# roryhighnam/iib_project_ldpc_codes

Hardware: AMD Instinct MI355X
Metric: decoded codewords/sec + info-bit Gb/s, (3,6) n=10k 50-iter BP, 1/2/4/8 MI355X (higher is better)
Workload: dtype f32

## Files before the change

iib_project_ldpc_codes_amd/_native.py:

```python
import ctypes as ct
import os

HERE = os.path.dirname(os.path.abspath(__file__))
LIB_PATH = os.environ.get("LDPC_LIB_PATH") or os.path.join(HERE, "libldpc_mi355x.so")

LDPC_OK = 0
LDPC_EINVAL, LDPC_ENODEV, LDPC_EHIP, LDPC_ENOMEM, LDPC_EUNSUP = -1, -2, -3, -4, -5
CH_BEC, CH_BSC, CH_AWGN = 0, 1, 2
ALGO_SPA, ALGO_MINSUM = 0, 1
MC_NCOUNT = 4
RM_TX, RM_PUNCT, RM_KNOWN = 0, 1, 2

_lib = None


class Quant(ct.Structure):
    _fields_ = [("scale", ct.c_float), ("msg_bits", ct.c_int32), ("post_bits", ct.c_int32),
                ("norm8", ct.c_int32), ("offset", ct.c_int32)]


class LdpcError(RuntimeError):
    def __init__(self, func, rc, msg):
        super().__init__(f"{func} failed ({rc}): {msg}")
        self.rc = rc
# ... 24 lines not shown
    "ldpc_bp_decode_batch_dev": ([P, P, i, i, i, f, i, P, P, P, P], i),
    "ldpc_channel_dev": ([i, f, u64, u64, i, i, P, P], i),
    "ldpc_mc_batch_dev": ([P, i, f, u64, u64, i, i, i, f, i, i, i64, P, P], i),
    "ldpc_last_error": ([], ct.c_char_p),
    "ldpc_device_count": ([], i),
    "ldpc_set_device": ([i], i),
    "ldpc_sync": ([P], i),
    "ldpc_bp_kernel_name": ([P, i], ct.c_char_p),
    "ldpc_debug_lane_layout": ([P, P, i, i, i, i, P, P, P, P], i),
    "ldpc_debug_irr_layout": ([P, P, P, P, i, i, P, P, P], i),
    "ldpc_debug_loc_layout": ([P, P, P, P, i, i, i, P, P, P, P], i),
    "ldpc_debug_loc_chain_layout": ([P, P, P, P, i, i, P, P, P, P, P], i),
    "ldpc_debug_loc_variant": ([P, P, P, P, i, i, i, P], i),
    "ldpc_debug_mc_plan": ([P, i64, i64, i64, i, i, P], i),
    "ldpc_debug_bp_plan": ([P, P, P, P, i, i, i, P, i, P, P], i),
    "ldpc_bp_layered_decode_batch_dev": ([P, P, i, i, i, f, i, P, P, P, P], i),
    "ldpc_mc_layered_batch_dev": ([P, i, f, u64, u64, i, i, i, f, i, i, i64, P, P], i),
    "ldpc_debug_layer_schedule": ([P, P, P, P, i, i, P, P], i),
    "ldpc_layer_rule": ([], ct.c_char_p),
    "ldpc_debug_layer_plan": ([P, P, P, P, i, i, i, P, i, P, P], i),
    "ldpc_bp_layered_q_decode_batch_dev": ([P, P, i, i, P, i, P, P, P, P], i),
    "ldpc_mc_layered_q_batch_dev": ([P, i, f, u64, u64, i, i, P, i, i, i64, P, P], i),
    "ldpc_debug_layer_q_plan": ([P, P, P, P, i, i, i, P, i, P, P], i),
    "ldpc_mc_layered_q_cw_batch_dev": ([P, P, P, i, f, f, u64, u64, i, i, P, i, i, i64, P, P], i),
    "ldpc_debug_layer_q_cw_plan": ([P, P, P, P, i, i, i, P, i, i, P, P], i),
    "ldpc_debug_qc_cw_plan": ([i, i, i, P, i, P, i, i, P, P], i),
    "ldpc_quant_check": ([P], i),
    "ldpc_graph_create_qc": ([i, i, i, P, ct.POINTER(P)], i),
    "ldpc_graph_layer_rule": ([P], ct.c_char_p),
    "ldpc_debug_qc_expand": ([i, i, i, P, P, P, P, P, P], i),
# ... 70 lines not shown
```

iib_project_ldpc_codes_amd/csrc/bp_dispatch.hip:

```cpp
#include "kernel_args.hpp"
#include "ldpc_mi355x.h"

namespace ldpc {

int device_cus() {
    int dev = 0, cus = 0;
    if (hipGetDevice(&dev) != hipSuccess ||
        hipDeviceGetAttribute(&cus, hipDeviceAttributeMultiprocessorCount, dev) != hipSuccess || cus <= 0)
        cus = 256;
    return cus;
}

const char *bp_kernel_name(const ldpc_graph &g, int early_stop) {
    return bp_plan(g, 1, 50, 0, early_stop != 0, false, early_stop != 2, device_cus()).name;
}

hipError_t FloodFamily::launch(const BpPlan &p, const SoftCall &c, float *scratch, hipStream_t s) const {
    BpArgs a = call_args<BpArgs>(c);
    a.cptr = g.cptr;
    a.cvar = g.cvar;
    a.vptr = g.vptr;
    a.vslot = g.vslot;
    a.n = g.n;
    a.m = g.m;
    a.E = g.E;
    a.scratch = scratch;
    a.scratch_bytes = p.scratch;
    const bool et = c.early_stop, mc = c.mc;
    switch (p.path) {
        case BpPath::Loc: return c.algo == 0 ? launch_loc_spa(p, g, a, et, mc, s) : launch_loc_ms(p, g, a, et, mc, s);
        case BpPath::Lds36: return launch_lds36(p, g, a, c.algo, et, mc, s);
        case BpPath::Irr: return launch_irr(p, g, a, c.algo, et, mc, s);
        case BpPath::None: return hipErrorInvalidValue;
        default: return launch_generic(p, g, a, c.algo, et, mc, s);
    }
}

hipError_t LayerFamily::launch(const BpPlan &p, const SoftCall &c, float *scratch, hipStream_t s) const {
    if (p.path == BpPath::None || !g.lay_tab || !g.lay_var) return hipErrorNotSupported;
    LayerArgs a = call_args<LayerArgs>(c);
    a.tab = g.lay_tab;
    a.var = g.lay_var;
// ... 40 lines not shown
```

iib_project_ldpc_codes_amd/csrc/bp_loc.hpp:

```cpp
#pragma once
#include "bp_device.hpp"

namespace ldpc {
namespace {

#ifndef LDPC_LOC_VGROUP
#define LDPC_LOC_VGROUP 1
#endif
#ifndef LDPC_LOC_CGROUP
#define LDPC_LOC_CGROUP 1
#endif
template <int N, int D>
__device__ __forceinline__ uint32_t bits_parity(const float2 (&x)[D], bool hi, uint32_t seed) {
    auto w = [&](int j) { return __float_as_uint(hi ? x[j].y : x[j].x); };
    uint32_t p = seed;
    int j = 2;
#pragma unroll
    for (; j + 1 < N; j += 2) p = xor3u(p, w(j), w(j + 1));
    if (j < N) p ^= w(j);
    return p;
}
template <int D, int ALGO, bool MIXED = false, bool SGN = false, int CL = 0>
__device__ __forceinline__ int loc_check_pair(float *msg, int W, int Nc, int i, float2 &l0, float2 &l1, float alpha,
                                              uint32_t lpar = 0u, float2 *chain = nullptr) {
// ... 53 lines not shown
__device__ __forceinline__ int loc_check_dispatch(int code, float *msg, int W, int Nc, int i, float2 &l0, float2 &l1,
                                                  float alpha, uint32_t lpar) {
    if constexpr (D == DHI) {
        if (code >> 8) return loc_check_pair<D, ALGO, true, SGN>(msg, W, Nc, i, l0, l1, alpha, lpar);
        return loc_check_pair<D, ALGO, false, SGN>(msg, W, Nc, i, l0, l1, alpha, lpar);
    } else {
        if (code == D) return loc_check_pair<D, ALGO, false, SGN>(msg, W, Nc, i, l0, l1, alpha, lpar);
        return loc_check_dispatch<D + 1, DHI, ALGO, SGN>(code, msg, W, Nc, i, l0, l1, alpha, lpar);
    }
}

template <typename V>
__device__ __forceinline__ V ld_fresh(const V *p, int idx) {
    asm volatile("" : "+v"(idx));
    return p[idx];
}

__device__ __forceinline__ bool block_any(int pred, uint32_t *flag, int par) {
    if (__builtin_amdgcn_ballot_w64(pred != 0) != 0 && (threadIdx.x & (kWave - 1)) == 0) flag[par] = 1u;
    __syncthreads();
    const bool any = flag[par] != 0u;
    if (threadIdx.x == 0) flag[par ^ 1] = 0u;
    return any;
}
__device__ __forceinline__ uint32_t block_count(int pred, uint32_t *flag, int par) {
    const uint64_t bal = __builtin_amdgcn_ballot_w64(pred != 0);
    if (bal != 0 && (threadIdx.x & (kWave - 1)) == 0) atomicAdd(&flag[par], (uint32_t)__popcll(bal));
    __syncthreads();
    const uint32_t c = flag[par];
    if (threadIdx.x == 0) flag[par ^ 1] = 0u;
// ... 23 lines not shown
    constexpr int VP = 2 * KP;
    constexpr int DVM = DVN0 > DVN1 ? DVN0 : DVN1;
    constexpr int DVA = DVM > 0 ? DVM : 1;
    constexpr int DVP = DVA;
    extern __shared__ __align__(16) unsigned char smem[];
    __shared__ uint32_t stop_flag[2];
    float *msg = reinterpret_cast<float *>(smem);
    const int tid = threadIdx.x;
    const int n = a.n, iters = a.max_iters;
    const int lpos0 = (int)((uint32_t)(size_t)(lds_u8 *)smem >> 2);
    const uint32_t base2 = (uint32_t)lpos0 | ((uint32_t)lpos0 << 16);
    constexpr bool SPA = ALGO == 0;
    constexpr bool INF0 = ABS0 || ALGO == 1, INF1 = ABS1 || ALGO == 1;
    uint32_t sp[VP][DVA];
    uint32_t inf[VP];
    auto load_sp = [&](int v, int u) {
        return (uint32_t)ld_fresh(a.loc_pos, (v * DVP + u) * T + tid) + base2;
    };
    auto load_vars = [&](int (&vv)[2 * VP]) {
#pragma unroll
        for (int i = 0; i < 2 * VP; ++i) vv[i] = ld_fresh(a.loc_var, i * T + tid);
    };
#pragma unroll
    for (int k = 0; k < KP; ++k) {
        if constexpr (INF0) inf[2 * k] = (uint32_t)a.loc_info[(2 * k) * T + tid];
        if constexpr (INF1) inf[2 * k + 1] = (uint32_t)a.loc_info[(2 * k + 1) * T + tid];
    }
    auto at = [](uint32_t ba) -> lds_f32 & { return *(lds_f32 *)(size_t)ba; };
    const float neutral = SPA ? 1.0f : 0.0f;

    auto gather = [&](auto dn_tag, auto abs_tag, int v, const uint32_t (&spv)[DVA], float2 (&cv)[DVA],
                      uint32_t (&a0)[DVA], uint32_t (&a1)[DVA]) {
        constexpr int DN = decltype(dn_tag)::value;
        constexpr bool AB = decltype(abs_tag)::value;
        const int nl = chained(v) ? DN - 1 : DN;
#pragma unroll
// ... 109 lines not shown
        if (per && tid == 0) next_b = round == 0 ? (int)atomicAdd(a.work, 1u) : (int)claim;
        __syncthreads();
        const int b = per ? __builtin_amdgcn_readfirstlane(next_b) : (int)blockIdx.x + round * (int)gridDim.x;
        if (b >= a.B) break;
        if (per && tid == 0) claim = atomicAdd(a.work, 1u);
        const uint64_t cw = a.first_cw + (uint64_t)b;
        int redo_it = -1;
    restart:
        int slab_it = -2;
        bool slab_now = false;
        if constexpr (ET) {
            if (tid == 0) stop_flag[0] = stop_flag[1] = 0u;
        }
        constexpr bool STG = CL > 0;
        auto load_tabs = [&]() {
#pragma unroll
            for (int k = 0; k < KP; ++k) {
#pragma unroll
                for (int u = 0; u < DVN0; ++u) sp[2 * k][u] = load_sp(2 * k, u);
#pragma unroll
                for (int u = 0; u < DVN1; ++u)
                    if (!(chained(2 * k + 1) && u == DVN1 - 1)) sp[2 * k + 1][u] = load_sp(2 * k + 1, u);
            }
        };
        int vv[2 * VP];
        if constexpr (STG) {
            load_tabs();
            load_vars(vv);
        }
        int err0 = 0;
        if constexpr (MC) {
            for (int i = tid; i <= iters; i += T) curve[i] = 0;
            if constexpr (MSET)
                for (int i = tid; i < nsw; i += T) syn[i] = 0u;
            for (int g4 = tid; g4 < (n + 3) >> 2; g4 += T) {
                const uint4 r = chan_block(a.ch, cw, g4);
#pragma unroll
                for (int q = 0; q < 4; ++q) {
                    if (4 * g4 + q >= n) break;
                    const float l = chan_soft_word(a.ch, r, q);
                    msg[4 * g4 + q] = to_msg<ALGO>(l);
                    err0 += (l < 0.0f);
                }
            }
        } else {
            if constexpr (MSET)
                for (int i = tid; i < nsw; i += T) syn[i] = 0u;
            if constexpr (STG) {
                float r[2 * VP];
                const float *lb = a.llr + (size_t)b * n;
                int t = tid;
                asm volatile("" : "+v"(t));
#pragma unroll
                for (int i = 0; i < 2 * VP; ++i) r[i] = lb[min(t + i * T, n - 1)];
#pragma unroll
                for (int i = 0; i < 2 * VP; ++i)
                    if (t + i * T < n) msg[t + i * T] = to_msg<ALGO>(r[i]);
            } else {
                for (int v = tid; v < n; v += T) msg[v] = to_msg<ALGO>(a.llr[(size_t)b * n + v]);
            }
        }
        __syncthreads();
        if constexpr (MC) {
            const int w = wave_sum(err0);
            if ((tid & (kWave - 1)) == 0) atomicAdd(&curve[0], w);
        }
        if constexpr (!STG) load_tabs();
        float2 L[VP];
        if constexpr (MC || STG) {
            if constexpr (!STG) load_vars(vv);
#pragma unroll
            for (int v = 0; v < VP; ++v)
                L[v] = make_float2(vv[2 * v] >= 0 ? msg[vv[2 * v]] : 0.0f, vv[2 * v + 1] >= 0 ? msg[vv[2 * v + 1]] : 0.0f);
        } else {
#pragma unroll
            for (int v = 0; v < VP; ++v) {
                const int v0 = ld_fresh(a.loc_var, (v * 2 + 0) * T + tid), v1 = ld_fresh(a.loc_var, (v * 2 + 1) * T + tid);
                L[v] = make_float2(v0 >= 0 ? msg[v0] : 0.0f, v1 >= 0 ? msg[v1] : 0.0f);
            }
        }
        __syncthreads();
        float2 loc[VP];
        auto init = [&](auto dn_tag, int v) {
            constexpr int DN = decltype(dn_tag)::value;
            float2 w;
// ... 264 lines not shown
                    if (v0 >= 0) msg[v0] = (hbits >> (2 * v)) & 1 ? -1.0f : 1.0f;
                    if (v1 >= 0) msg[v1] = (hbits >> (2 * v + 1)) & 1 ? -1.0f : 1.0f;
                }
                __syncthreads();
                if (a.hard)
                    for (int v = tid; v < n; v += T) a.hard[(size_t)b * n + v] = (uint8_t)(msg[v] < 0.0f);
                if (a.its && tid == 0) a.its[b] = it;
                continue;
            }
        }
        constexpr bool FIX = !ET && !MC;
        float2 pr[VP];
        int pid[2 * VP];
        bool clamped = false;
        if constexpr (FIX) {
            load_vars(pid);
            if constexpr (SPA) {
#pragma unroll
                for (int v = 0; v < VP; ++v)
                    clamped |= fabsf(__builtin_amdgcn_logf(L[v].x)) >= 125.5f || fabsf(__builtin_amdgcn_logf(L[v].y)) >= 125.5f;
            }
        }
        auto post = [&](auto dn_tag, auto abs_tag, auto subst_tag, int v) {
            constexpr int DN = decltype(dn_tag)::value;
            constexpr bool SUBST = decltype(subst_tag)::value;
            uint32_t a0[DVA], a1[DVA], spv[DVA];
            float2 cv[DVA];
            if constexpr (FIX) {
                gather(dn_tag, abs_tag, v, sp[v], cv, a0, a1);
            } else {
#pragma unroll
// ... 29 lines not shown
        };
        if (FIX && SPA && __builtin_expect(__builtin_amdgcn_ballot_w64(clamped) != 0, 0)) {
#pragma unroll
            for (int k = 0; k < KP; ++k) {
                post(int_c<DVN0>{}, bool_c<ABS0>{}, bool_c<true>{}, 2 * k);
                post(int_c<DVN1>{}, bool_c<ABS1>{}, bool_c<true>{}, 2 * k + 1);
            }
        } else {
#pragma unroll
            for (int k = 0; k < KP; ++k) {
                post(int_c<DVN0>{}, bool_c<ABS0>{}, bool_c<false>{}, 2 * k);
                post(int_c<DVN1>{}, bool_c<ABS1>{}, bool_c<false>{}, 2 * k + 1);
            }
        }
        __syncthreads();
#pragma unroll
        for (int v = 0; v < VP; ++v) {
            int v0, v1;
            if constexpr (FIX) {
                v0 = pid[2 * v];
                v1 = pid[2 * v + 1];
            } else {
                v0 = ld_fresh(a.loc_var, (v * 2 + 0) * T + tid);
                v1 = ld_fresh(a.loc_var, (v * 2 + 1) * T + tid);
            }
            if (v0 >= 0) msg[v0] = pr[v].x;
            if (v1 >= 0) msg[v1] = pr[v].y;
        }
        __syncthreads();
        if constexpr (FIX) {
            float o[2 * VP];
            int t = tid;
            asm volatile("" : "+v"(t));
#pragma unroll
            for (int i = 0; i < 2 * VP; ++i) o[i] = msg[min(t + i * T, n - 1)];
#pragma unroll
            for (int i = 0; i < 2 * VP; ++i) {
                const int v = t + i * T;
                if (v < n) {
                    if (a.post) a.post[(size_t)b * n + v] = o[i] * Domain<ALGO>::out;
                    if (a.hard) a.hard[(size_t)b * n + v] = (uint8_t)(o[i] < 0.0f);
                }
            }
        } else {
            for (int v = tid; v < n; v += T) {
                const float s = msg[v];
                if (a.post) a.post[(size_t)b * n + v] = s * Domain<ALGO>::out;
                if (a.hard) a.hard[(size_t)b * n + v] = (uint8_t)(s < 0.0f);
            }
        }
        if (a.its && tid == 0) a.its[b] = iters;
    }
}

template <int DLO, int DHI, int D0, int D1, bool A0, bool A1, int T, int KP, int ALGO, bool ET, bool MC>
hipError_t launch_loc_shape(const BpPlan &p, BpArgs a, hipStream_t s) {
// ... 78 lines not shown
```

iib_project_ldpc_codes_amd/csrc/bp_plan.cpp:

```cpp
#include "ldpc_internal.hpp"

#ifndef LDPC_LDS36_MINSUM
#define LDPC_LDS36_MINSUM 1
#endif
#ifndef LDPC_LOC
#define LDPC_LOC 1
#endif
#ifndef LDPC_LOC_CHAIN
#define LDPC_LOC_CHAIN 1
#endif
#ifndef LDPC_LOC_MSMC
#define LDPC_LOC_MSMC 1
#endif
#ifndef LDPC_LOC_HARD_ET
#define LDPC_LOC_HARD_ET 1
#endif
#ifndef LDPC_LOC_ET_POST
#define LDPC_LOC_ET_POST 1
#endif
#ifndef LDPC_LOC_PERSIST
#define LDPC_LOC_PERSIST 1
#endif
#ifndef LDPC_LDS36_GRID
#define LDPC_LDS36_GRID 256
#endif
#ifndef LDPC_GMEM_GRID
#define LDPC_GMEM_GRID 256
#endif
#ifndef LDPC_GMEM_HYB
#define LDPC_GMEM_HYB 1
#endif

namespace ldpc {
namespace {

size_t loc_lds_bytes(const GraphShape &g, int iters, bool mc, bool syn) {
    return pad16((size_t)std::max(g.loc_words + 64, g.n) * 4) + (mc ? curve_bytes(iters) : 0) +
           (syn ? (size_t)((g.m + 31) / 32) * 4 : 0);
}
size_t loc_ep_slab_bytes(const GraphShape &g) { return (size_t)(2 * g.loc_KP) * (size_t)g.loc_T * 2 * 4; }

size_t irr_lds_bytes(const GraphShape &g, int iters) {
    const int nsyn = (g.m + 31) >> 5;
    return pad16((size_t)g.irr_S * 4) + (size_t)((nsyn + 3) & ~3) * 4 + (size_t)(iters + 1) * 4;
}
bool irr_slab(const GraphShape &g) { return g.irr_S < g.irr_P; }

size_t lds36_bytes(const GraphShape &g, int iters, bool et, bool mc) {
    const size_t Ep = (size_t)lds_pair_span(g.m, 6) + kLdsDummy;
    size_t s = Ep * 4;
    if (et || mc) s = pad16(Ep * 5);
    if (mc) s += (size_t)(iters + 1) * 4;
// ... 4 lines not shown
size_t generic_lds_bytes(const GraphShape &g, int iters, bool mc) {
    return generic_msg_bytes(g) + (mc ? (size_t)(iters + 1) * 4 : 0);
}

void gmem_plan(BpPlan &p, size_t fixed, size_t E) {
    p.threads = LDPC_GMEM_T;
    const size_t room = fixed < kLdsMax - 4096 ? kLdsMax - 4096 - fixed : 0;
    p.lds_slots = LDPC_GMEM_HYB ? (int)std::min(E, room / 4) : 0;
    p.lds = fixed + (size_t)p.lds_slots * 4;
}

BpPath choose_path(const GraphShape &g, int iters, bool et, bool mc, int algo, bool hard_only) {
    if (!g.consistent) return BpPath::None;
    const bool lds36_ms = LDPC_LDS36_MINSUM && algo == 1 && g.lane_T && g.dv == 3 && g.dc == 6 && g.loc_T != 512;
    const bool one_cls = loc_variant(g) == kLocReg36;
    const bool ep_ok = LDPC_LOC_ET_POST && (size_t)std::max(g.loc_words + 64, g.n) * 4 >= (size_t)g.n * 5;
    const bool mode_ok = mc ? (algo == 0 || (LDPC_LOC_MSMC && one_cls))
                            : (!et || (LDPC_LOC_HARD_ET && (hard_only || ep_ok) && (algo == 0 || one_cls)));
    const bool mset = et && algo == 1;
    if (LDPC_LOC && mode_ok && iters > 0 && !lds36_ms && loc_variant(g) != kLocNone &&
        loc_lds_bytes(g, iters, mc || mset, mset) <= kLdsMax - 2048)
        return BpPath::Loc;
    if (g.lane_T && g.dv == 3 && g.dc == 6 && lds36_bytes(g, iters, et, mc) <= kLdsMax - 2048)
        return BpPath::Lds36;
    if (g.irr_VPT && irr_lds_bytes(g, iters) <= kLdsMax - 1024) return BpPath::Irr;
    const int d = g.max_cdeg;
    if (d > 32) return BpPath::None;
    const bool lds = generic_lds_bytes(g, iters, mc) <= kLdsMax - 2048;
    if (d <= 8) return lds ? BpPath::Generic8 : BpPath::GenericG8;
    if (d <= 16) return lds ? BpPath::Generic16 : BpPath::GenericG16;
    return lds ? BpPath::Generic32 : BpPath::GenericG32;
}

}

BpPlan bp_plan(const GraphShape &g, int B, int iters, int algo, bool et, bool mc, bool want_post, int cus) {
    algo = algo ? 1 : 0;
    BpPlan p;
    p.path = choose_path(g, iters, et, mc, algo, !want_post);
    p.grid = B;
    size_t slab_per_wg = 0;
    switch (p.path) {
        case BpPath::Loc: {
            p.name = "bp_loc_kernel";
            p.threads = g.loc_T;
            const bool mset = et && algo == 1;
            p.lds = loc_lds_bytes(g, iters, mc || mset, mset);
            p.chain = LDPC_LOC_CHAIN && g.chn_Tq > 0 && algo == 0 && !et && !mc;
            if (p.chain) p.lds = pad16((size_t)std::max(g.chn_words + 64, g.n) * 4);
            const bool ep = et && !mc && want_post;
            p.persistent = ep || ((et || LDPC_LOC_PERSIST > 1) && LDPC_LOC_PERSIST);
            if (p.persistent) p.grid = std::min(B, 2 * cus);
            if (ep) slab_per_wg = loc_ep_slab_bytes(g);
            break;
        }
        case BpPath::Lds36:
            p.name = "bp_lds_kernel<3,6>";
            p.threads = g.lane_T;
            p.lds = lds36_bytes(g, iters, et, mc);
            if (et || (LDPC_LDS36_PREFETCH && !mc)) p.grid = std::min(B, LDPC_LDS36_GRID);
            break;
        case BpPath::Irr:
            p.name = irr_slab(g) ? "bp_irr_kernel<lds+slab>" : "bp_irr_kernel<lds>";
            p.threads = kIrrT;
// ... 20 lines not shown
                                                    : "bp_generic_kernel<32,gmem>";
            p.grid = std::min(B, LDPC_GMEM_GRID);
            gmem_plan(p, mc ? curve_bytes(iters) : 0, (size_t)g.E);
            slab_per_wg = generic_msg_bytes(g);
            break;
        }
        default: return p;
    }
    p.slab = slab_per_wg * (size_t)p.grid;
    p.scratch = p.slab;
    if (p.persistent) {
        p.counter = (long)p.slab;
        p.scratch += sizeof(uint32_t);
    }
    return p;
}

BpPlan bp_ens_plan(int n, int dv, int dc, int B, int iters, int , bool , bool mc,
                   bool , int cus) {
    BpPlan p;
    if (n <= 0 || dv <= 0 || dc <= 1 || dc > 32) return p;
    const size_t E = (size_t)n * (size_t)dv;
    const size_t block = ens_block_bytes((size_t)n, E), syn = ens_syn_bytes(E / (size_t)dc);
    const bool lds = block + syn + (mc ? (size_t)(iters + 1) * 4 : 0) <= kLdsMax - 2048;
    const int w = dc <= 8 ? 0 : (dc <= 16 ? 1 : 2);
    static const BpPath paths[2][3] = {{BpPath::EnsG8, BpPath::EnsG16, BpPath::EnsG32},
                                       {BpPath::Ens8, BpPath::Ens16, BpPath::Ens32}};
    static const char *const names[2][3] = {{"bp_ens_kernel<8,gmem>", "bp_ens_kernel<16,gmem>", "bp_ens_kernel<32,gmem>"},
                                            {"bp_ens_kernel<8,lds>", "bp_ens_kernel<16,lds>", "bp_ens_kernel<32,lds>"}};
    p.grid = std::min(B, std::min(cus, LDPC_GMEM_GRID));
// ... 87 lines not shown
```

iib_project_ldpc_codes_amd/csrc/capi.cpp:

```cpp
#include <cmath>
#include <cstdio>
#include <cstdlib>
#include <algorithm>
#include <cstring>
#include <memory>
#include <mutex>
#include <string>
#include <vector>

#include "encode_host.hpp"
#include "graph_device.hpp"
#include "rate_match_host.hpp"
#include "workspace.hpp"

namespace ldpc {
namespace {
thread_local std::string g_err;
std::mutex g_mu;
DropInCache g_dropin;

LayoutOptions layout_options(int loc_T = 0) {
    LayoutOptions opt;
    const char *noloc = getenv("LDPC_NO_LOC_LAYOUT");
    opt.loc_layout = !(noloc && noloc[0] == '1');
// ... 55 lines not shown
    host_layouts(h, g, L, true, layout_options());
    if (need_schedule && g.lay_L <= 0) {
        set_error(kNoSchedule);
        return LDPC_EUNSUP;
    }
    return write_plans(count, calls, out, names, col4, no_plan,
                       [&](int B, int iters, int algo, bool et, bool mc, bool want_post) {
                           return plan(g, B, iters, algo, et, mc, want_post, cus);
                       });
}

static SoftCall decode_call(int B, int max_iters, int algo, float alpha, int early_stop, const float *llr, void *post,
                            uint8_t *hard, int32_t *its) {
    SoftCall c{B, max_iters, algo, alpha, early_stop != 0, false};
    c.llr = llr, c.post = post, c.hard = hard, c.its = its;
    return c;
}
static SoftCall mc_call(int B, int max_iters, int algo, float alpha, int early_stop, const ChanArgs &ch,
                        uint64_t first_cw) {
    SoftCall c{B, max_iters, algo, alpha, early_stop != 0, true};
    c.ch = ch, c.first_cw = first_cw;
    return c;
}

template <typename Family>
static int soft_launch(Workspace &ws, const Family &f, const SoftCall &c, hipStream_t s) {
    const BpPlan p = f.plan(c, device_cus());
    float *scratch = p.scratch ? ws.scratch.get<float>((p.scratch + 3) / 4) : nullptr;
    LDPC_ALLOCATED(scratch || !p.scratch);
    if (p.scratch > (scratch ? ws.scratch.cap : 0)) LDPC_HIP(hipErrorInvalidValue);
// ... 184 lines not shown
    LDPC_TRY(host_graph_from_csr(check_ptr, check_var, var_ptr, var_slot, n, m, h));
    *variant = kLocNone;
    if (!h.consistent) return LDPC_OK;
    GraphShape g;
    HostLayouts L;
    host_layouts(h, g, L, true, layout_options(T));
    *variant = loc_variant(g);
    return LDPC_OK;
}

int ldpc_debug_bp_plan(const int32_t *check_ptr, const int32_t *check_var, const int32_t *var_ptr,
                       const int32_t *var_slot, int n, int m, int count, const int32_t *calls, int cus, int64_t *out,
                       char *names) {
    return graph_plans(check_ptr, check_var, var_ptr, var_slot, n, m, count, calls, cus, out, names, bp_plan, false,
                       &BpPlan::lds_slots);
}

int ldpc_debug_bec_plan(int n, int m, int dc, int count, const int32_t *calls, int64_t *out, char *names) {
    LDPC_REQUIRE(n > 0 && m > 0 && dc >= 0 && count >= 0 && (count == 0 || (calls && out && names)),
                 "bad plan arguments");
    for (int i = 0; i < count; ++i) {
        const int32_t *c = calls + 4 * (size_t)i;
        LDPC_REQUIRE(c[0] >= 0 && c[0] <= 2 && c[1] >= 0 && c[2] >= 0, "bad plan arguments");
        const BecPlan p = bec_plan(n, m, dc, c[1], c[2], static_cast<BecMode>(c[0]), c[3]);
        int64_t *o = out + 9 * (size_t)i;
        o[0] = (int64_t)p.kernel; o[1] = p.threads; o[2] = p.W; o[3] = p.plane; o[4] = p.cw_per_wg;
        o[5] = p.grid; o[6] = (int64_t)p.lds; o[7] = p.F; o[8] = (int64_t)p.cap;
        snprintf(names + 64 * (size_t)i, 64, "%s", p.name);
    }
    return LDPC_OK;
// ... 977 lines not shown
```

iib_project_ldpc_codes_amd/csrc/kernel_args.hpp:

```cpp
#pragma once
#include "device_common.hpp"
#include "ldpc_internal.hpp"

namespace ldpc {

struct BecArgs {
    const int32_t *cvar, *cptr, *vptr, *vchk;
    int n, m, dv, dc;
    uint8_t *words;
    int32_t *errors, *its;
    int max_iters;
    ChanArgs ch;
    uint64_t first_cw;
    int32_t *trial;
    int64_t graph_stride;
};

struct BpArgs {
    const int32_t *cptr, *cvar, *vptr, *vslot;
    int n, m, E, B;
    const float *llr;
    float *post;
    uint8_t *hard;
    int32_t *its;
    int max_iters;
    float alpha;
    ChanArgs ch;
    uint64_t first_cw;
    int32_t *trial;
    float *scratch;
    size_t scratch_bytes;
    const int32_t *lane_var, *lane_slot;
    int lds_slots;
    const int32_t *irr_lane, *irr_cdeg;
    int irr_KC, irr_S, irr_P;
    const int32_t *loc_var, *loc_pos, *loc_info;
    int loc_P, loc_ncls, loc_words;
    int loc_cls_q[5], loc_cls_d[4], loc_cls_w[5];
    uint32_t *work;
};

struct EnsArgs {
    const int32_t *chk, *var;
    int n, m, dv, dc, E, B;
    const float *llr;
    float *post;
    uint8_t *hard;
    int32_t *its;
// ... 104 lines not shown
```

iib_project_ldpc_codes_amd/csrc/ldpc_internal.hpp:

```cpp
#pragma once
#include <hip/hip_runtime.h>
#include <stdint.h>

#include <algorithm>
#include <string>
#include <vector>

#include "kernel_shapes.hpp"

struct ldpc_quant;

struct GraphShape {
    int n = 0, m = 0, k = 0, E = 0;
    int dv = 0, dc = 0;
    int max_vdeg = 0, max_cdeg = 0;
    bool consistent = false;
    int vchk_len = 0;
    int lane_T = 0, lane_VPT = 0;
    int irr_VPT = 0, irr_KC = 0, irr_DC = 0, irr_S = 0, irr_P = 0;
    int loc_T = 0, loc_KP = 0, loc_DVN = 0, loc_P = 0, loc_ncls = 0, loc_words = 0, loc_dlo = 0, loc_dhi = 0;
    int loc_dvn0 = 0, loc_dvn1 = 0;
    bool loc_abs0 = false, loc_abs1 = false;
    int loc_cls_q[5] = {0}, loc_cls_d[4] = {0}, loc_cls_w[5] = {0};
    int chn_Tq = 0, chn_words = 0;
// ... 103 lines not shown
constexpr size_t kLdsMax = 160 * 1024;
constexpr size_t kBecWordLdsCap = kLdsMax - 1024, kPeelLdsCap = kLdsMax - 1024;
constexpr size_t kBecBitsLdsCap = kLdsMax - 4096, kBecBitsWideLdsCap = 72 * 1024;
constexpr int kLdsDummy = 3 * 32 + 4;

inline int lds_pair_pos(int slot, int dc) {
    const int c = slot / dc, j = slot % dc;
    return (c >> 1) * 2 * dc + 2 * j + (c & 1);
}
inline int lds_pair_span(int m, int dc) { return ((m + 1) / 2) * 2 * dc; }

namespace ldpc {

void set_error(const std::string &msg);
constexpr size_t pad16(size_t b) { return (b + 15) & ~(size_t)15; }

enum class BecMode { Decode, Mc, EnsMc };
enum class BecKernel { Word, DecBits, McBits, Peel, None };
struct BecPlan {
    BecKernel kernel = BecKernel::None;
    const char *name = "none";
    int threads = 0;
    int W = 0, plane = 0;
    int cw_per_wg = 0;
    int64_t grid = 0;
    size_t lds = 0;
    size_t cap = 0;
    int F = 0;
};
BecPlan bec_plan(int n, int m, int dc, int B, int iters, BecMode mode, int peel_cap);
// ... 24 lines not shown

enum class BpPath {
    Loc, Lds36, Irr, Generic8, Generic16, Generic32, GenericG8, GenericG16, GenericG32, None,
    Ens8, Ens16, Ens32, EnsG8, EnsG16, EnsG32,
    Layer8, Layer16, Layer32, LayerG8, LayerG16, LayerG32,
    LayerQ8, LayerQ16, LayerQ32,
    QcQ64x8, QcQ64x16, QcQ64x32, QcQ256x8, QcQ256x16, QcQ256x32
};
struct BpPlan {
    BpPath path = BpPath::None;
    const char *name = "none";
    int threads = 0, grid = 0;
    size_t lds = 0;
    int lds_slots = 0;
    bool chain = false;
    bool persistent = false;
    size_t slab = 0;
    long counter = -1;
    size_t scratch = 0;
    int wg_per_cu = 0;
};
BpPlan bp_plan(const GraphShape &g, int B, int iters, int algo, bool early_stop, bool mc, bool want_post, int cus);
BpPlan bp_ens_plan(int n, int dv, int dc, int B, int iters, int algo, bool early_stop, bool mc, bool want_post,
                   int cus);
BpPlan bp_layer_plan(const GraphShape &g, int B, int iters, int algo, bool early_stop, bool mc, bool want_post,
                     int cus);
BpPlan bp_layer_q_plan(const GraphShape &g, int B, int iters, int algo, bool early_stop, bool mc, bool want_post,
                       int cus);
BpPlan bp_layer_q_cw_plan(const GraphShape &g, int B, int iters, bool mc, bool cw);
constexpr size_t layer_q_plane_bytes(size_t n) { return 4 * ((n + 31) / 32); }
constexpr size_t layer_q_record_bytes(int max_cdeg) { return max_cdeg <= 16 ? 4 : 8; }
constexpr size_t layer_block_bytes(size_t n, size_t E) { return pad16((n + E) * 4); }
constexpr int kLayerMaxD = 32, kLayerTab = kLayerMaxD + 1;
constexpr int kQcRow = 1 + 2 * kLayerMaxD;
constexpr size_t ens_block_bytes(size_t n, size_t E) { return pad16(E * 8 + n * 4); }
constexpr size_t generic_block_bytes(size_t n, size_t E) { return pad16(E * 5 + n * 4); }
constexpr size_t curve_bytes(int iters) { return pad16((size_t)(iters + 1) * 4); }
// ... 12 lines not shown
    c.p2 = p2;
    c.k0 = (uint32_t)seed;
    c.k1 = (uint32_t)(seed >> 32);
    return c;
}

struct SoftCall {
    int B = 0, max_iters = 0, algo = 0;
    float alpha = 1.0f;
    bool early_stop = false;
    bool mc = false;
    const float *llr = nullptr;
    void *post = nullptr;
    uint8_t *hard = nullptr;
    int32_t *its = nullptr;
    ChanArgs ch{};
    uint64_t first_cw = 0;
    int32_t *trial = nullptr;
    bool cw_mode = false;
    const uint8_t *cw = nullptr;
    const uint8_t *rm = nullptr;
    float known_llr = 0.0f;
};

struct FloodFamily {
    const ldpc_graph &g;
    BpPlan plan(const SoftCall &c, int cus) const {
        return bp_plan(g, c.B, c.max_iters, c.algo, c.early_stop, c.mc, c.post != nullptr, cus);
    }
    hipError_t launch(const BpPlan &p, const SoftCall &c, float *scratch, hipStream_t s) const;
};
struct EnsFamily {
    int n, dv, dc;
    const int32_t *chk, *var;
    BpPlan plan(const SoftCall &c, int cus) const {
        return bp_ens_plan(n, dv, dc, c.B, c.max_iters, c.algo, c.early_stop, c.mc, c.post != nullptr, cus);
    }
    hipError_t launch(const BpPlan &p, const SoftCall &c, float *scratch, hipStream_t s) const;
};
struct LayerFamily {
    const ldpc_graph &g;
    BpPlan plan(const SoftCall &c, int cus) const {
        return bp_layer_plan(g, c.B, c.max_iters, c.algo, c.early_stop, c.mc, c.post != nullptr, cus);
// ... 125 lines not shown
```

iib_project_ldpc_codes_amd/csrc/loc_layout.cpp:

```cpp
#include <algorithm>
#include <cmath>
#include <cstdlib>
#include <cstdint>
#include <deque>
#include <vector>

#include "ldpc_internal.hpp"

#ifndef LDPC_LOC_SEARCH
#define LDPC_LOC_SEARCH 10
#endif
#ifndef LDPC_LOC_T0
#define LDPC_LOC_T0 0.0
#endif

namespace {
bool assign(const std::vector<std::vector<int>> &adj, std::vector<int> cap, int NR, std::vector<int> &to) {
    const int NL = (int)adj.size();
    std::vector<std::vector<int>> held(NR);
    std::vector<int> order(NL);
    to.assign(NL, -1);
    for (int v = 0; v < NL; ++v) order[v] = v;
    std::stable_sort(order.begin(), order.end(), [&](int a, int b) { return adj[a].size() < adj[b].size(); });
    for (int v : order)
// ... 596 lines not shown
        uint32_t info = 0;
        int u = 0, jl = 0;
        for (int j = 0; j < DV; ++j) {
            const int e = vslot[vptr[v] + j];
            if (slot_check[e] == c) { jl = j; continue; }
            if (urow[e] < 0) continue;
            int32_t &pk = C.pos[((size_t)vi * DVN + u) * T + t];
            pk = (int32_t)(((uint32_t)pk & ~(0xFFFFu << (16 * h))) | ((uint32_t)cw[e] << (16 * h)));
            info |= 1u << (u + 4 * h);
            ++u;
        }
        info |= (uint32_t)jl << (8 + 2 * h);
        info |= 1u << (16 + 4 * h + jl);
        C.info[(size_t)vi * T + t] |= (int32_t)info;
    }
    return true;
}
```

include/ldpc_mi355x.h:

```cpp
#ifndef LDPC_MI355X_H
#define LDPC_MI355X_H

#include <stdint.h>

#ifdef __cplusplus
extern "C" {
#endif

#define LDPC_OK 0
#define LDPC_EINVAL (-1)
#define LDPC_ENODEV (-2)
#define LDPC_EHIP (-3)
#define LDPC_ENOMEM (-4)
#define LDPC_EUNSUP (-5)

#define LDPC_CH_BEC 0
#define LDPC_CH_BSC 1
#define LDPC_CH_AWGN 2

#define LDPC_ALGO_SPA 0
#define LDPC_ALGO_MINSUM 1

int message_passing(int *Mvc, int iterations, int *variable_to_check_list,
                    int *check_to_variable_list, int *errors, int n, int k, int dv, int dc);
// ... 154 lines not shown
int ldpc_debug_irr_layout(const int32_t *check_ptr, const int32_t *check_var, const int32_t *var_ptr,
                          const int32_t *var_slot, int n, int m, int32_t *shape, int32_t *lane, int32_t *cdeg);

int ldpc_debug_loc_layout(const int32_t *check_ptr, const int32_t *check_var, const int32_t *var_ptr,
                          const int32_t *var_slot, int n, int m, int T, int32_t *shape, int32_t *var, int32_t *pos,
                          int32_t *info);

int ldpc_debug_loc_chain_layout(const int32_t *check_ptr, const int32_t *check_var, const int32_t *var_ptr,
                                const int32_t *var_slot, int n, int m, int32_t *shape, int32_t *var, int32_t *pos,
                                int32_t *info, int32_t *chk);

int ldpc_debug_bp_plan(const int32_t *check_ptr, const int32_t *check_var, const int32_t *var_ptr,
                       const int32_t *var_slot, int n, int m, int count, const int32_t *calls, int cus, int64_t *out,
                       char *names);

int ldpc_debug_ens_plan(int n, int dv, int dc, int count, const int32_t *calls, int cus, int64_t *out,
                        char *names);

int ldpc_debug_layer_schedule(const int32_t *check_ptr, const int32_t *check_var, const int32_t *var_ptr,
                              const int32_t *var_slot, int n, int m, int32_t *num_layers, int32_t *layer);
const char *ldpc_layer_rule(void);

int ldpc_debug_layer_plan(const int32_t *check_ptr, const int32_t *check_var, const int32_t *var_ptr,
                          const int32_t *var_slot, int n, int m, int count, const int32_t *calls, int cus,
                          int64_t *out, char *names);

int ldpc_debug_layer_q_plan(const int32_t *check_ptr, const int32_t *check_var, const int32_t *var_ptr,
                            const int32_t *var_slot, int n, int m, int count, const int32_t *calls, int cus,
                            int64_t *out, char *names);
int ldpc_quant_check(const ldpc_quant *q);
// ... 42 lines not shown
```

Baseline: 2.567 million.

## Use buffer loads and 128-bit vectorized LLR/posterior I/O in local BP kernel

Adds a wide_io plan flag, set when the local path runs without early stop or Monte Carlo and the pointers are aligned. With it, the kernel loads LLRs and stores posteriors and hard bits as 16-byte or packed 4-byte vectors. Table reads and the remaining I/O switch to raw buffer loads and stores, whose hardware range checks replace per-element bounds branches, and active-lane guards replace per-variable sign checks. A layout check now requires the padding lanes to be exactly those at or beyond Tq, and LDS sizing requires spare slack so that clamped out-of-range stores stay in bounds. The aim is fewer memory instructions and branches at kernel entry and exit, at the cost of stricter layout and alignment conditions.

New measurement: 2.615 million, median of 6. +1.9%, better.

```diff
diff --git a/iib_project_ldpc_codes_amd/_native.py b/iib_project_ldpc_codes_amd/_native.py
--- a/iib_project_ldpc_codes_amd/_native.py
+++ b/iib_project_ldpc_codes_amd/_native.py
@@ -62,6 +62,7 @@
     "ldpc_debug_loc_variant": ([P, P, P, P, i, i, i, P], i),
     "ldpc_debug_mc_plan": ([P, i64, i64, i64, i, i, P], i),
     "ldpc_debug_bp_plan": ([P, P, P, P, i, i, i, P, i, P, P], i),
+    "ldpc_debug_bp_plan_io": ([P, P, P, P, i, i, i, P, i, P, P], i),
     "ldpc_bp_layered_decode_batch_dev": ([P, P, i, i, i, f, i, P, P, P, P], i),
     "ldpc_mc_layered_batch_dev": ([P, i, f, u64, u64, i, i, i, f, i, i, i64, P, P], i),
     "ldpc_debug_layer_schedule": ([P, P, P, P, i, i, P, P], i),
diff --git a/iib_project_ldpc_codes_amd/csrc/bp_dispatch.hip b/iib_project_ldpc_codes_amd/csrc/bp_dispatch.hip
--- a/iib_project_ldpc_codes_amd/csrc/bp_dispatch.hip
+++ b/iib_project_ldpc_codes_amd/csrc/bp_dispatch.hip
@@ -26,6 +26,7 @@
     a.E = g.E;
     a.scratch = scratch;
     a.scratch_bytes = p.scratch;
+    a.wide_io = p.wide_io;
     const bool et = c.early_stop, mc = c.mc;
     switch (p.path) {
         case BpPath::Loc: return c.algo == 0 ? launch_loc_spa(p, g, a, et, mc, s) : launch_loc_ms(p, g, a, et, mc, s);
diff --git a/iib_project_ldpc_codes_amd/csrc/bp_loc.hpp b/iib_project_ldpc_codes_amd/csrc/bp_loc.hpp
--- a/iib_project_ldpc_codes_amd/csrc/bp_loc.hpp
+++ b/iib_project_ldpc_codes_amd/csrc/bp_loc.hpp
@@ -91,6 +91,14 @@
 __device__ __forceinline__ V ld_fresh(const V *p, int idx) {
     asm volatile("" : "+v"(idx));
     return p[idx];
+}
+typedef float f32x4 __attribute__((ext_vector_type(4)));
+typedef uint32_t u32x4 __attribute__((ext_vector_type(4)));
+__device__ __forceinline__ __amdgpu_buffer_rsrc_t row_rsrc(const void *row, int bytes) {
+    return __builtin_amdgcn_make_buffer_rsrc(const_cast<void *>(row), 0, bytes, 0x00020000);
+}
+__device__ __forceinline__ int32_t ld_row(__amdgpu_buffer_rsrc_t tab, int entry, uint32_t lane_bytes) {
+    return (int32_t)__builtin_amdgcn_raw_buffer_load_b32(tab, lane_bytes, 4 * entry, 0);
 }
 
 __device__ __forceinline__ bool block_any(int pred, uint32_t *flag, int par) {
@@ -144,12 +152,22 @@
     constexpr bool INF0 = ABS0 || ALGO == 1, INF1 = ABS1 || ALGO == 1;
     uint32_t sp[VP][DVA];
     uint32_t inf[VP];
-    auto load_sp = [&](int v, int u) {
-        return (uint32_t)ld_fresh(a.loc_pos, (v * DVP + u) * T + tid) + base2;
+    auto lane_bytes = [&]() {
+        uint32_t l = 4u * (uint32_t)tid;
+        asm volatile("" : "+v"(l));
+        return l;
+    };
+    auto load_sp = [&](int v, int u, uint32_t lane4 = 0u) {
+        if constexpr (CL > 0) return (uint32_t)ld_row(row_rsrc(a.loc_pos, VP * DVP * T * 4), (v * DVP + u) * T, lane4) + base2;
+        else return (uint32_t)ld_fresh(a.loc_pos, (v * DVP + u) * T + tid) + base2;
     };
     auto load_vars = [&](int (&vv)[2 * VP]) {
 #pragma unroll
         for (int i = 0; i < 2 * VP; ++i) vv[i] = ld_fresh(a.loc_var, i * T + tid);
+    };
+    auto load_vars_row = [&](int (&vv)[2 * VP], uint32_t lane4) {
+#pragma unroll
+        for (int i = 0; i < 2 * VP; ++i) vv[i] = ld_row(row_rsrc(a.loc_var, 2 * VP * T * 4), i * T, lane4);
     };
 #pragma unroll
     for (int k = 0; k < KP; ++k) {
@@ -289,19 +307,20 @@
         }
         constexpr bool STG = CL > 0;
         auto load_tabs = [&]() {
+            const uint32_t lane4 = CL > 0 ? lane_bytes() : 0u;
 #pragma unroll
             for (int k = 0; k < KP; ++k) {
 #pragma unroll
-                for (int u = 0; u < DVN0; ++u) sp[2 * k][u] = load_sp(2 * k, u);
+                for (int u = 0; u < DVN0; ++u) sp[2 * k][u] = load_sp(2 * k, u, lane4);
 #pragma unroll
                 for (int u = 0; u < DVN1; ++u)
-                    if (!(chained(2 * k + 1) && u == DVN1 - 1)) sp[2 * k + 1][u] = load_sp(2 * k + 1, u);
+                    if (!(chained(2 * k + 1) && u == DVN1 - 1)) sp[2 * k + 1][u] = load_sp(2 * k + 1, u, lane4);
             }
         };
         int vv[2 * VP];
         if constexpr (STG) {
             load_tabs();
-            load_vars(vv);
+            load_vars_row(vv, lane_bytes());
         }
         int err0 = 0;
         if constexpr (MC) {
@@ -322,15 +341,29 @@
             if constexpr (MSET)
                 for (int i = tid; i < nsw; i += T) syn[i] = 0u;
             if constexpr (STG) {
-                float r[2 * VP];
-                const float *lb = a.llr + (size_t)b * n;
-                int t = tid;
+                const __amdgpu_buffer_rsrc_t rl = row_rsrc(a.llr + (size_t)b * n, 4 * n);
+                uint32_t t = (uint32_t)tid;
                 asm volatile("" : "+v"(t));
-#pragma unroll
-                for (int i = 0; i < 2 * VP; ++i) r[i] = lb[min(t + i * T, n - 1)];
-#pragma unroll
-                for (int i = 0; i < 2 * VP; ++i)
-                    if (t + i * T < n) msg[t + i * T] = to_msg<ALGO>(r[i]);
+                if (a.wide_io) {
+                    f32x4 r[VP / 2];
+#pragma unroll
+                    for (int j = 0; j < VP / 2; ++j)
+                        r[j] = __builtin_bit_cast(f32x4, __builtin_amdgcn_raw_buffer_load_b128(rl, 16u * (t + j * T), 0, 0));
+#pragma unroll
+                    for (int j = 0; j < VP / 2; ++j) {
+                        f32x4 w;
+                        w.x = to_msg<ALGO>(r[j].x); w.y = to_msg<ALGO>(r[j].y);
+                        w.z = to_msg<ALGO>(r[j].z); w.w = to_msg<ALGO>(r[j].w);
+                        *reinterpret_cast<f32x4 *>(msg + min(4u * (t + j * T), (uint32_t)n)) = w;
+                    }
+                } else {
+                    float r[2 * VP];
+#pragma unroll
+                    for (int i = 0; i < 2 * VP; ++i)
+                        r[i] = __uint_as_float(__builtin_amdgcn_raw_buffer_load_b32(rl, 4u * (t + i * T), 0, 0));
+#pragma unroll
+                    for (int i = 0; i < 2 * VP; ++i) msg[min(t + i * T, (uint32_t)n)] = to_msg<ALGO>(r[i]);
+                }
             } else {
                 for (int v = tid; v < n; v += T) msg[v] = to_msg<ALGO>(a.llr[(size_t)b * n + v]);
             }
@@ -342,8 +375,15 @@
         }
         if constexpr (!STG) load_tabs();
         float2 L[VP];
-        if constexpr (MC || STG) {
-            if constexpr (!STG) load_vars(vv);
+        if constexpr (STG) {
+#pragma unroll
+            for (int v = 0; v < VP; ++v) L[v] = make_float2(0.0f, 0.0f);
+            if (tid < a.loc_cls_q[1]) {
+#pragma unroll
+                for (int v = 0; v < VP; ++v) L[v] = make_float2(msg[vv[2 * v]], msg[vv[2 * v + 1]]);
+            }
+        } else if constexpr (MC) {
+            load_vars(vv);
 #pragma unroll
             for (int v = 0; v < VP; ++v)
                 L[v] = make_float2(vv[2 * v] >= 0 ? msg[vv[2 * v]] : 0.0f, vv[2 * v + 1] >= 0 ? msg[vv[2 * v + 1]] : 0.0f);
@@ -638,7 +678,7 @@
         int pid[2 * VP];
         bool clamped = false;
         if constexpr (FIX) {
-            load_vars(pid);
+            load_vars_row(pid, lane_bytes());
             if constexpr (SPA) {
 #pragma unroll
                 for (int v = 0; v < VP; ++v)
@@ -698,32 +738,70 @@
             }
         }
         __syncthreads();
-#pragma unroll
-        for (int v = 0; v < VP; ++v) {
-            int v0, v1;
-            if constexpr (FIX) {
-                v0 = pid[2 * v];
-                v1 = pid[2 * v + 1];
-            } else {
-                v0 = ld_fresh(a.loc_var, (v * 2 + 0) * T + tid);
-                v1 = ld_fresh(a.loc_var, (v * 2 + 1) * T + tid);
-            }
-            if (v0 >= 0) msg[v0] = pr[v].x;
-            if (v1 >= 0) msg[v1] = pr[v].y;
+        if constexpr (FIX && CL > 0) {
+            if (tid < a.loc_cls_q[1]) {
+#pragma unroll
+                for (int v = 0; v < VP; ++v) {
+                    msg[pid[2 * v]] = pr[v].x;
+                    msg[pid[2 * v + 1]] = pr[v].y;
+                }
+            }
+        } else if constexpr (FIX) {
+#pragma unroll
+            for (int v = 0; v < VP; ++v) {
+                msg[min((uint32_t)pid[2 * v], (uint32_t)n)] = pr[v].x;
+                msg[min((uint32_t)pid[2 * v + 1], (uint32_t)n)] = pr[v].y;
+            }
+        } else {
+#pragma unroll
+            for (int v = 0; v < VP; ++v) {
+                const int v0 = ld_fresh(a.loc_var, (v * 2 + 0) * T + tid);
+                const int v1 = ld_fresh(a.loc_var, (v * 2 + 1) * T + tid);
+                if (v0 >= 0) msg[v0] = pr[v].x;
+                if (v1 >= 0) msg[v1] = pr[v].y;
+            }
         }
         __syncthreads();
         if constexpr (FIX) {
-            float o[2 * VP];
-            int t = tid;
+            uint32_t t = (uint32_t)tid;
             asm volatile("" : "+v"(t));
-#pragma unroll
-            for (int i = 0; i < 2 * VP; ++i) o[i] = msg[min(t + i * T, n - 1)];
-#pragma unroll
-            for (int i = 0; i < 2 * VP; ++i) {
-                const int v = t + i * T;
-                if (v < n) {
-                    if (a.post) a.post[(size_t)b * n + v] = o[i] * Domain<ALGO>::out;
-                    if (a.hard) a.hard[(size_t)b * n + v] = (uint8_t)(o[i] < 0.0f);
+            if (a.wide_io) {
+                f32x4 o[VP / 2];
+#pragma unroll
+                for (int j = 0; j < VP / 2; ++j)
+                    o[j] = *reinterpret_cast<const f32x4 *>(msg + min(4u * (t + j * T), (uint32_t)n));
+                if (a.post) {
+                    const __amdgpu_buffer_rsrc_t rp = row_rsrc(a.post + (size_t)b * n, 4 * n);
+#pragma unroll
+                    for (int j = 0; j < VP / 2; ++j)
+                        __builtin_amdgcn_raw_buffer_store_b128(__builtin_bit_cast(u32x4, o[j] * Domain<ALGO>::out), rp,
+                                                               16u * (t + j * T), 0, 0);
+                }
+                if (a.hard) {
+                    const __amdgpu_buffer_rsrc_t rh = row_rsrc(a.hard + (size_t)b * n, n);
+#pragma unroll
+                    for (int j = 0; j < VP / 2; ++j) {
+                        const uint32_t h = (uint32_t)(o[j].x < 0.0f) | (uint32_t)(o[j].y < 0.0f) << 8 |
+                                           (uint32_t)(o[j].z < 0.0f) << 16 | (uint32_t)(o[j].w < 0.0f) << 24;
+                        __builtin_amdgcn_raw_buffer_store_b32(h, rh, 4u * (t + j * T), 0, 0);
+                    }
+                }
+            } else {
+                float o[2 * VP];
+#pragma unroll
+                for (int i = 0; i < 2 * VP; ++i) o[i] = msg[min(t + i * T, (uint32_t)n)];
+                if (a.post) {
+                    const __amdgpu_buffer_rsrc_t rp = row_rsrc(a.post + (size_t)b * n, 4 * n);
+#pragma unroll
+                    for (int i = 0; i < 2 * VP; ++i)
+                        __builtin_amdgcn_raw_buffer_store_b32(__float_as_uint(o[i] * Domain<ALGO>::out), rp,
+                                                              4u * (t + i * T), 0, 0);
+                }
+                if (a.hard) {
+                    const __amdgpu_buffer_rsrc_t rh = row_rsrc(a.hard + (size_t)b * n, n);
+#pragma unroll
+                    for (int i = 0; i < 2 * VP; ++i)
+                        __builtin_amdgcn_raw_buffer_store_b8((uint8_t)(o[i] < 0.0f), rh, t + i * T, 0, 0);
                 }
             }
         } else {
diff --git a/iib_project_ldpc_codes_amd/csrc/bp_plan.cpp b/iib_project_ldpc_codes_amd/csrc/bp_plan.cpp
--- a/iib_project_ldpc_codes_amd/csrc/bp_plan.cpp
+++ b/iib_project_ldpc_codes_amd/csrc/bp_plan.cpp
@@ -35,7 +35,7 @@
 namespace {
 
 size_t loc_lds_bytes(const GraphShape &g, int iters, bool mc, bool syn) {
-    return pad16((size_t)std::max(g.loc_words + 64, g.n) * 4) + (mc ? curve_bytes(iters) : 0) +
+    return pad16(loc_msg_words(g.loc_words, g.n) * 4) + (mc ? curve_bytes(iters) : 0) +
            (syn ? (size_t)((g.m + 31) / 32) * 4 : 0);
 }
 size_t loc_ep_slab_bytes(const GraphShape &g) { return (size_t)(2 * g.loc_KP) * (size_t)g.loc_T * 2 * 4; }
@@ -70,11 +70,11 @@
     if (!g.consistent) return BpPath::None;
     const bool lds36_ms = LDPC_LDS36_MINSUM && algo == 1 && g.lane_T && g.dv == 3 && g.dc == 6 && g.loc_T != 512;
     const bool one_cls = loc_variant(g) == kLocReg36;
-    const bool ep_ok = LDPC_LOC_ET_POST && (size_t)std::max(g.loc_words + 64, g.n) * 4 >= (size_t)g.n * 5;
+    const bool ep_ok = LDPC_LOC_ET_POST && loc_msg_words(g.loc_words, g.n) * 4 >= (size_t)g.n * 5;
     const bool mode_ok = mc ? (algo == 0 || (LDPC_LOC_MSMC && one_cls))
                             : (!et || (LDPC_LOC_HARD_ET && (hard_only || ep_ok) && (algo == 0 || one_cls)));
     const bool mset = et && algo == 1;
-    if (LDPC_LOC && mode_ok && iters > 0 && !lds36_ms && loc_variant(g) != kLocNone &&
+    if (LDPC_LOC && mode_ok && iters > 0 && !lds36_ms && loc_variant(g) != kLocNone && loc_spare_ok(g.loc_words, g.n) &&
         loc_lds_bytes(g, iters, mc || mset, mset) <= kLdsMax - 2048)
         return BpPath::Loc;
     if (g.lane_T && g.dv == 3 && g.dc == 6 && lds36_bytes(g, iters, et, mc) <= kLdsMax - 2048)
@@ -102,8 +102,8 @@
             p.threads = g.loc_T;
             const bool mset = et && algo == 1;
             p.lds = loc_lds_bytes(g, iters, mc || mset, mset);
-            p.chain = LDPC_LOC_CHAIN && g.chn_Tq > 0 && algo == 0 && !et && !mc;
-            if (p.chain) p.lds = pad16((size_t)std::max(g.chn_words + 64, g.n) * 4);
+            p.chain = LDPC_LOC_CHAIN && g.chn_Tq > 0 && algo == 0 && !et && !mc && loc_spare_ok(g.chn_words, g.n);
+            if (p.chain) p.lds = pad16(loc_msg_words(g.chn_words, g.n) * 4);
             const bool ep = et && !mc && want_post;
             p.persistent = ep || ((et || LDPC_LOC_PERSIST > 1) && LDPC_LOC_PERSIST);
             if (p.persistent) p.grid = std::min(B, 2 * cus);
@@ -154,6 +154,13 @@
         p.scratch += sizeof(uint32_t);
     }
     return p;
+}
+
+bool bp_wide_io(const BpPlan &p, const GraphShape &g, bool early_stop, bool mc, const void *llr, const void *post,
+                const void *hard, bool narrow) {
+    auto aligned = [](const void *q, uintptr_t to) { return (reinterpret_cast<uintptr_t>(q) & (to - 1)) == 0; };
+    return p.path == BpPath::Loc && !early_stop && !mc && !narrow && g.n % 4 == 0 && aligned(llr, 16) &&
+           aligned(post, 16) && aligned(hard, 4);
 }
 
 BpPlan bp_ens_plan(int n, int dv, int dc, int B, int iters, int , bool , bool mc,
diff --git a/iib_project_ldpc_codes_amd/csrc/capi.cpp b/iib_project_ldpc_codes_amd/csrc/capi.cpp
--- a/iib_project_ldpc_codes_amd/csrc/capi.cpp
+++ b/iib_project_ldpc_codes_amd/csrc/capi.cpp
@@ -93,6 +93,8 @@
                             uint8_t *hard, int32_t *its) {
     SoftCall c{B, max_iters, algo, alpha, early_stop != 0, false};
     c.llr = llr, c.post = post, c.hard = hard, c.its = its;
+    const char *nowide = getenv("LDPC_NO_WIDE_IO");
+    c.narrow_io = nowide && nowide[0] == '1';
     return c;
 }
 static SoftCall mc_call(int B, int max_iters, int algo, float alpha, int early_stop, const ChanArgs &ch,
@@ -307,6 +309,32 @@
                        char *names) {
     return graph_plans(check_ptr, check_var, var_ptr, var_slot, n, m, count, calls, cus, out, names, bp_plan, false,
                        &BpPlan::lds_slots);
+}
+
+int ldpc_debug_bp_plan_io(const int32_t *check_ptr, const int32_t *check_var, const int32_t *var_ptr,
+                          const int32_t *var_slot, int n, int m, int count, const int64_t *calls, int cus, int64_t *out,
+                          char *names) {
+    LDPC_REQUIRE(count >= 0 && (count == 0 || (calls && out && names)) && cus > 0, "bad plan arguments");
+    HostGraph h;
+    LDPC_TRY(host_graph_from_csr(check_ptr, check_var, var_ptr, var_slot, n, m, h));
+    GraphShape g;
+    HostLayouts L;
+    host_layouts(h, g, L, true, layout_options());
+    for (int i = 0; i < count; ++i) {
+        const int64_t *c = calls + 9 * (size_t)i;
+        LDPC_REQUIRE(c[0] >= 0 && c[1] >= 0, "bad plan arguments");
+        const bool et = c[3] != 0, mc = c[4] != 0;
+        BpPlan p = bp_plan(g, (int)c[0], (int)c[1], (int)c[2], et, mc, c[6] != 0, cus);
+        p.wide_io = bp_wide_io(p, g, et, mc, reinterpret_cast<const void *>(c[5]), reinterpret_cast<const void *>(c[6]),
+                               reinterpret_cast<const void *>(c[7]), c[8] != 0);
+        int64_t *o = out + 11 * (size_t)i;
+        o[0] = (int64_t)p.path; o[1] = p.threads; o[2] = p.grid; o[3] = (int64_t)p.lds; o[4] = p.lds_slots;
+        o[5] = p.persistent; o[6] = (int64_t)p.slab; o[7] = p.counter; o[8] = (int64_t)p.scratch;
+        o[9] = p.wide_io;
+        o[10] = p.path == BpPath::Loc ? (int64_t)loc_msg_words(p.chain ? g.chn_words : g.loc_words, g.n) : 0;
+        snprintf(names + 64 * (size_t)i, 64, "%s", p.name);
+    }
+    return LDPC_OK;
 }
 
 int ldpc_debug_bec_plan(int n, int m, int dc, int count, const int32_t *calls, int64_t *out, char *names) {
diff --git a/iib_project_ldpc_codes_amd/csrc/kernel_args.hpp b/iib_project_ldpc_codes_amd/csrc/kernel_args.hpp
--- a/iib_project_ldpc_codes_amd/csrc/kernel_args.hpp
+++ b/iib_project_ldpc_codes_amd/csrc/kernel_args.hpp
@@ -32,6 +32,7 @@
     size_t scratch_bytes;
     const int32_t *lane_var, *lane_slot;
     int lds_slots;
+    int wide_io;
     const int32_t *irr_lane, *irr_cdeg;
     int irr_KC, irr_S, irr_P;
     const int32_t *loc_var, *loc_pos, *loc_info;
diff --git a/iib_project_ldpc_codes_amd/csrc/ldpc_internal.hpp b/iib_project_ldpc_codes_amd/csrc/ldpc_internal.hpp
--- a/iib_project_ldpc_codes_amd/csrc/ldpc_internal.hpp
+++ b/iib_project_ldpc_codes_amd/csrc/ldpc_internal.hpp
@@ -141,6 +141,9 @@
 
 void set_error(const std::string &msg);
 constexpr size_t pad16(size_t b) { return (b + 15) & ~(size_t)15; }
+constexpr int kLocSpare = 4;
+constexpr size_t loc_msg_words(int words, int n) { return (size_t)(words + 64 > n ? words + 64 : n); }
+constexpr bool loc_spare_ok(int words, int n) { return words + 64 >= n + kLocSpare; }
 
 enum class BecMode { Decode, Mc, EnsMc };
 enum class BecKernel { Word, DecBits, McBits, Peel, None };
@@ -195,6 +198,7 @@
     size_t lds = 0;
     int lds_slots = 0;
     bool chain = false;
+    bool wide_io = false;
     bool persistent = false;
     size_t slab = 0;
     long counter = -1;
@@ -202,6 +206,8 @@
     int wg_per_cu = 0;
 };
 BpPlan bp_plan(const GraphShape &g, int B, int iters, int algo, bool early_stop, bool mc, bool want_post, int cus);
+bool bp_wide_io(const BpPlan &p, const GraphShape &g, bool early_stop, bool mc, const void *llr, const void *post,
+                const void *hard, bool narrow);
 BpPlan bp_ens_plan(int n, int dv, int dc, int B, int iters, int algo, bool early_stop, bool mc, bool want_post,
                    int cus);
 BpPlan bp_layer_plan(const GraphShape &g, int B, int iters, int algo, bool early_stop, bool mc, bool want_post,
@@ -244,6 +250,7 @@
     void *post = nullptr;
     uint8_t *hard = nullptr;
     int32_t *its = nullptr;
+    bool narrow_io = false;
     ChanArgs ch{};
     uint64_t first_cw = 0;
     int32_t *trial = nullptr;
@@ -256,7 +263,9 @@
 struct FloodFamily {
     const ldpc_graph &g;
     BpPlan plan(const SoftCall &c, int cus) const {
-        return bp_plan(g, c.B, c.max_iters, c.algo, c.early_stop, c.mc, c.post != nullptr, cus);
+        BpPlan p = bp_plan(g, c.B, c.max_iters, c.algo, c.early_stop, c.mc, c.post != nullptr, cus);
+        p.wide_io = bp_wide_io(p, g, c.early_stop, c.mc, c.llr, c.post, c.hard, c.narrow_io);
+        return p;
     }
     hipError_t launch(const BpPlan &p, const SoftCall &c, float *scratch, hipStream_t s) const;
 };
diff --git a/iib_project_ldpc_codes_amd/csrc/loc_layout.cpp b/iib_project_ldpc_codes_amd/csrc/loc_layout.cpp
--- a/iib_project_ldpc_codes_amd/csrc/loc_layout.cpp
+++ b/iib_project_ldpc_codes_amd/csrc/loc_layout.cpp
@@ -634,5 +634,8 @@
         info |= 1u << (16 + 4 * h + jl);
         C.info[(size_t)vi * T + t] |= (int32_t)info;
     }
+    for (int t = 0; t < T; ++t)
+        for (int i = 0; i < 2 * VP; ++i)
+            if ((C.var[(size_t)i * T + t] >= 0) != (t < Tq)) return false;
     return true;
 }
diff --git a/include/ldpc_mi355x.h b/include/ldpc_mi355x.h
--- a/include/ldpc_mi355x.h
+++ b/include/ldpc_mi355x.h
@@ -192,6 +192,10 @@
                        const int32_t *var_slot, int n, int m, int count, const int32_t *calls, int cus, int64_t *out,
                        char *names);
 
+int ldpc_debug_bp_plan_io(const int32_t *check_ptr, const int32_t *check_var, const int32_t *var_ptr,
+                          const int32_t *var_slot, int n, int m, int count, const int64_t *calls, int cus, int64_t *out,
+                          char *names);
+
 int ldpc_debug_ens_plan(int n, int dv, int dc, int count, const int32_t *calls, int cus, int64_t *out,
                         char *names);
 
```
